# ktiwary2/nerf_pl

Measured on AMD Instinct MI355X. Metric: rays/sec (64c+128f) Blender-lego 400^2 training step, higher is better.
Workload: dtype f16x3

## Files before the change

### __graft_entry__.py

```python
import os
import subprocess
import sys

REPO = os.path.dirname(os.path.abspath(__file__))


def build() -> None:
    jobs = str(min(16, os.cpu_count() or 1))
    subprocess.run(["make", "-C", REPO, "-j", jobs], check=True)
    r = subprocess.run(["make", "-C", REPO, "-j", jobs, "asan"], check=False)
    if r.returncode != 0:
        print(f"build(): optional `make asan` failed (rc {r.returncode}); "
              "tests/test_abi_asan.py will skip", file=sys.stderr)
    if REPO not in sys.path:
        sys.path.insert(0, REPO)
    import nerf_pl_amd
    from nerf_pl_amd import (_lib, _lib_mesh, _lib_mesh_normals, _lib_optim, _lib_posegrad,
                             _lib_raygrad)
    missing = (_lib.missing_symbols() + _lib_mesh.missing_symbols()
               + _lib_mesh_normals.missing_symbols() + _lib_raygrad.missing_symbols()
               + _lib_posegrad.missing_symbols() + _lib_optim.missing_symbols())
    if missing:
        raise RuntimeError(f"libnerf_pl_amd.so lacks {missing}")


def smoke() -> None:
    if REPO not in sys.path:
        sys.path.insert(0, REPO)
    import torch
    from nerf_pl_amd import Embedding, NeRF, ReplayRNG, render_rays
    from nerf_pl_amd.rays import blender_rays
    from oracle import nerf_oracle as O

    dev = torch.device("cuda", 0)
    n_rays, S, I = 64, 32, 32
    rays = blender_rays(16, 1, near=2.0, far=6.0)[:n_rays].contiguous()
    g = torch.Generator().manual_seed(0)
    draws = [torch.rand(n_rays, S, generator=g), torch.randn(n_rays, S, generator=g),
             torch.rand(n_rays, I, generator=g), torch.rand(n_rays, I, generator=g),
             torch.randn(n_rays, S + I, generator=g)]
    params = [O.make_params(1, sigma_bias=0.5), O.make_params(2, sigma_bias=0.5)]
    ocap, cap = {}, {}
    ref = O.render_rays(params, rays, S, False, 1.0, 1.0, I, 32768, False,
                        rng=O.ReplayRNG(draws), capture=ocap)
    models = []
    for p in params:
        m = NeRF()
        m.load_state_dict(p)
        models.append(m.to(dev))
    res = render_rays(models, [Embedding(3, 10), Embedding(3, 4)], rays.to(dev), S, False, 1.0,
                      1.0, I, 32768, False, rng=ReplayRNG(draws), _capture=cap)
    pairs = [(res[k], ref[k]) for k in ref] + \
        [(cap[w], ocap[w]) for w in ("weights_coarse", "weights_fine")]
    worst = max((a.detach().cpu() - b).abs().max().item() for a, b in pairs)
# ... 16 lines not shown
```

### nerf_pl_amd/csrc/mlp_fwd3.hip

```cpp
#include "x3.h"

namespace {

using namespace x3;

constexpr int kHeadBytes = NR_H_SIZE * 4;
constexpr int kHeadDma = (kHeadBytes + 1023) / 1024;
constexpr int kHeadLds = kHeadDma * 1024;
#define NR_PE_REGS (NR_F16 || NR_BF1)
constexpr int kPeQ = 12;
constexpr int kPeBytes = NR_PE_REGS ? 0 : kWaves * kPeQ * 64 * 16;
constexpr int kNS = 2;
constexpr int kBlocks = kWaves;
constexpr int kLdsBytes = kRingBytes + kHeadLds + kPeBytes;
static_assert(kLdsBytes <= 160 * 1024, "LDS budget");

constexpr int kL1 = 0, kL2 = 4, kL3 = 20, kL4 = 36, kL5 = 52, kL6 = 72, kL7 = 88, kL8 = 104;
constexpr int kFinal = 120, kDir = 136, kQAll = 145, kQSigma = 120;

struct FwdTab {
    __host__ __device__ static constexpr int64_t off(int q) {
        return (int64_t)kHeadBytes + (int64_t)q * kSlotBytes;
    }
    __host__ __device__ static constexpr int sg(int q) { return q < kDir ? q / 2 : kDir / 2 + (q - kDir); }
    __host__ __device__ static constexpr int first(int G) { return G < kDir / 2 ? 2 * G : kDir + (G - kDir / 2); }
    __host__ __device__ static constexpr int size(int G) { return G < kDir / 2 ? 2 : 1; }
};
static_assert(FwdTab::off(kQAll) == (NR_F16 ? 2388000 : (NR_BF1 ? 1200160 : 3575840)),
              "packed size must match packing.fwd3_offsets()");

template <bool RELU, int NF, int NS>
__device__ __forceinline__ void head_dot(const f32x4 (&acc)[NF][NS], const float* __restrict__ w,
                                         int g, float (&p)[2]) {
    p[0] = p[1] = 0.f;
#pragma unroll
    for (int F = 0; F < NF; ++F) {
        const f32x4 v = *reinterpret_cast<const f32x4*>(w + 16 * F + 4 * g);
#pragma unroll
        for (int S = 0; S < NS; ++S)
#pragma unroll
            for (int r = 0; r < 4; ++r) p[S] = fmaf(RELU ? relu_keep(acc[F][S][r]) : acc[F][S][r], v[r], p[S]);
    }
#pragma unroll
    for (int S = 0; S < NS; ++S) p[S] = sum_over_groups(p[S]);
}

__device__ __forceinline__ void pe_encode(float (&pe)[16], float px, float py, float pz, int g) {
#pragma unroll
    for (int s = 0; s < 2; ++s)
#pragma unroll
        for (int i = 0; i < 4; ++i) {
            const int m = 4 * (4 * s + g) + i;
            const int k = (m * 11) >> 5;
            const int c = m - 3 * k;
            const float v = c == 0 ? px : (c == 1 ? py : pz);
            float sn, cs;
            sincosf(v * __uint_as_float((uint32_t)(127 + k) << 23), &sn, &cs);
            pe[8 * s + i] = sn;
            pe[8 * s + 4 + i] = cs;
        }
    if (g == 3) {
        pe[10] = px; pe[11] = py; pe[14] = pz; pe[15] = 0.f;
    }
}

__device__ __forceinline__ void pe_gather(float (&pe)[16], const float* __restrict__ row, int g) {
#pragma unroll
    for (int s = 0; s < 2; ++s)
#pragma unroll
        for (int i = 0; i < 4; ++i) {
            const int m = min(4 * (4 * s + g) + i, 29);
            const int k = (m * 11) >> 5;
            const int c = m - 3 * k;
            pe[8 * s + i] = row[3 + 6 * k + c];
            pe[8 * s + 4 + i] = row[6 + 6 * k + c];
        }
    if (g == 3) {
        pe[10] = row[0]; pe[11] = row[1]; pe[14] = row[2]; pe[15] = 0.f;
    }
}

__device__ __forceinline__ void dir_encode(float (&d)[8], float dx, float dy, float dz, int g) {
    const float sc = __uint_as_float((uint32_t)(127 + g) << 23);
    sincosf(dx * sc, &d[0], &d[4]);
    sincosf(dy * sc, &d[1], &d[5]);
    sincosf(dz * sc, &d[2], &d[6]);
    d[3] = g == 0 ? dx : (g == 1 ? dy : (g == 2 ? dz : 0.f));
    d[7] = 0.f;
}

__device__ __forceinline__ void dir_gather(float (&d)[8], const float* __restrict__ row, int g) {
#pragma unroll
    for (int c = 0; c < 3; ++c) {
        d[c] = row[3 + 6 * g + c];
        d[4 + c] = row[6 + 6 * g + c];
    }
    d[3] = g < 3 ? row[min(g, 2)] : 0.f;
    d[7] = 0.f;
}

template <int W, bool ROWS>
__device__ __forceinline__ void store_pe4(const float* v, int s, int jh, int S, int g,
                                          float* __restrict__ blk, int lane) {
    const int T = 2 * s + (g >> 1), gp = 2 * (g & 1) + jh;
#if NR_BF1
    store_slot(f32x4{v[0], v[1], v[2], v[3]}, blk, (T * 2 + S) * 64 + 16 * gp + (lane & 15));
#else
    if constexpr (ROWS)
        *reinterpret_cast<f32x4*>(blk + (16 * S + (lane & 15)) * W + 16 * T + 4 * gp) =
            f32x4{v[0], v[1], v[2], v[3]};
    else
        *reinterpret_cast<f32x4*>(blk + ((T * 2 + S) * 64 + 16 * gp + (lane & 15)) * 4) =
            f32x4{v[0], v[1], v[2], v[3]};
#endif
}

enum FwdMode { FWD_RAYS = 0, FWD_EMB = 1, FWD_PTS = 2 };

template <bool SAVE, bool ROWS>
struct PeSide {
    static constexpr int before(int T) { return SAVE ? (T > 2) + (T > 6) : 0; }
// ... 4 lines not shown
    __device__ __forceinline__ void operator()(GC, int t) const {
        if constexpr (SAVE) {
            if (t == 2 || t == 6) {
                const int u = 2 * GC::value + (t == 6), S = u >> 2, s = (u >> 1) & 1, jh = u & 1;
                store_pe4<64, ROWS>(&pe[S][8 * s + 4 * jh], s, jh, S, g, dst, lane);
            }
        }
    }
};

template <bool SAVE>
struct DirPeSide {
    static constexpr int before(int T) { return SAVE ? T / 2 : 0; }
    const float (&dpe)[kNS][8];
    float* dst;
    int g, lane;
    template <typename GC>
    __device__ __forceinline__ void operator()(GC, int t) const {
        if constexpr (SAVE) {
            if (t & 1) {
                const int u = t >> 1;
                store_pe4<32, true>(&dpe[u >> 1][4 * (u & 1)], 0, u & 1, u >> 1, g, dst, lane);
            }
        }
    }
};

struct Fwd3Args {
    const char* packed;
    const float* pts; const float* rays; const float* z; const float* x;
    int n, spr, xstride;
    float* out; float* save;
    const int32_t* slist; const int32_t* scount;
};

template <bool RELU, bool STORE, bool MASK, bool SIG, bool ROWS = true>
struct AccU {
    static constexpr bool kStores = STORE;
    static constexpr bool kPaired = STORE && ROWS && kRowPair;
    template <typename P> __device__ __forceinline__ void begin(const P&) {}
    const f32x4 (&X)[16][kNS];
    float* dst;
    uint32_t* msk;
    const float* wsig;
    int lane, g;
    float pend[2] = {0.f, 0.f};
    f32x4 held = {0.f, 0.f, 0.f, 0.f};
    uint32_t w[4] = {0u, 0u, 0u, 0u};
    float sig[2] = {0.f, 0.f};
    f32x2 wsg[2][4];
    __device__ __forceinline__ f32x2 wsig_of(int s, int p) const {
        return *reinterpret_cast<const f32x2*>(wsig + 32 * s + 16 * (p >> 1) + 4 * g + 2 * (p & 1));
    }
    __device__ __forceinline__ void preload() {
        if constexpr (SIG)
#pragma unroll
            for (int p = 0; p < 4; ++p) wsg[0][p] = wsig_of(0, p);
    }
    template <typename SC>
    __device__ __forceinline__ void operator()(SC, int sb, int p, float& x0, float& x1) {
        constexpr int s = SC::value;
        x0 = acc_b(X, s, sb, 2 * p);
        x1 = acc_b(X, s, sb, 2 * p + 1);
        if constexpr (RELU) { x0 = relu_unscale(x0); x1 = relu_unscale(x1); }
        else if constexpr (kWScale != 0) { x0 *= kWUnscale; x1 *= kWUnscale; }
        if constexpr (SIG) {
// ... 25 lines not shown
            }
        }
    }
};

template <int N>
struct PeU {
    static constexpr bool kStores = false;
    static constexpr bool kPaired = false;
    template <typename P> __device__ __forceinline__ void begin(const P&) {}
    const float (&pe)[kNS][N];
    template <typename SC>
    __device__ __forceinline__ void operator()(SC, int sb, int p, float& x0, float& x1) const {
        constexpr int s = SC::value;
        x0 = pe[sb][8 * s + 2 * p];
        x1 = pe[sb][8 * s + 2 * p + 1];
    }
};

template <int S = 0, typename GetU>
__device__ __forceinline__ void drain_all(GetU& u) {
    if constexpr (S < 8) {
#pragma unroll
        for (int sb = 0; sb < kNS; ++sb)
#pragma unroll
            for (int p = 0; p < 4; ++p) {
                float x0, x1;
                u(IC<S>(), sb, p, x0, x1);
            }
        drain_all<S + 1>(u);
    }
}

template <int MODE, bool SIGMA_ONLY, bool SAVE, bool LIST = false>
__global__ void __launch_bounds__(64 * kWaves, 1) mlp_fwd3_kernel(Fwd3Args a) {
    constexpr bool EMB = MODE == FWD_EMB;
    constexpr int QEND = SIGMA_ONLY ? kQSigma : kQAll;
    static_assert(!LIST || (SAVE && MODE == FWD_RAYS), "a listed run saves, on the ray path");
    __shared__ __attribute__((aligned(16))) char smem[kLdsBytes];
    const int lane = threadIdx.x & 63;
    const int wave = __builtin_amdgcn_readfirstlane(threadIdx.x >> 6);
    const int g = lane >> 4;
    const int blk = blockIdx.x * kBlocks + wave;
    const int m = LIST ? __builtin_amdgcn_readfirstlane(*a.scount) : a.n;
    if (LIST && (int)blockIdx.x * kBlocks * 32 >= m) return;
    int smp[2];
    bool valid[2];
#pragma unroll
    for (int S = 0; S < kNS; ++S) {
        const int s_raw = blk * 32 + 16 * S + (lane & 15);
        valid[S] = s_raw < m;
        if constexpr (LIST) smp[S] = a.slist[valid[S] ? s_raw : 0];
        else smp[S] = valid[S] ? s_raw : a.n - 1;
    }
    const char* P = a.packed;

    float pe[kNS][16], dg[kNS][8];
    float in[kNS][7];
#pragma unroll
    for (int S = 0; S < kNS; ++S) {
        const int s = smp[S];
        if constexpr (EMB) {
            pe_gather(pe[S], a.x + (size_t)s * a.xstride, g);
            if constexpr (!SIGMA_ONLY) dir_gather(dg[S], a.x + (size_t)s * a.xstride + NR_XYZ_CH, g);
        } else if constexpr (MODE == FWD_PTS) {
#pragma unroll
            for (int c = 0; c < 3; ++c) in[S][c] = a.pts[(size_t)s * 3 + c];
        } else {
            const float* r = a.rays + (size_t)(s / a.spr) * 8;
#pragma unroll
            for (int c = 0; c < 6; ++c) in[S][c] = r[c];
            in[S][6] = a.z[s];
        }
    }

    float* Hs = reinterpret_cast<float*>(smem + kRingBytes);
    const Dma dma = make_dma(P, FwdTab::off(kQAll), smem, wave, lane);
#pragma unroll
    for (int i = wave; i < kHeadDma; i += kWaves)
        __builtin_amdgcn_raw_ptr_buffer_load_lds(
            dma.rsrc, (__attribute__((address_space(3))) void*)(smem + kRingBytes + i * 1024), 16,
            dma.voff, i * 1024, 0, 0);
    prologue<FwdTab, QEND>(dma);
    const float* H = Hs;
    const int nb = (int)nr_blocks_pad(a.n);
    float* const SV = a.save;

    [[maybe_unused]] f32x4* pe_lds =
        reinterpret_cast<f32x4*>(smem + kRingBytes + kHeadLds) + wave * kPeQ * 64 + lane;
#pragma unroll
    for (int S = 0; S < kNS; ++S) {
        if constexpr (MODE == FWD_PTS) {
            pe_encode(pe[S], in[S][0], in[S][1], in[S][2], g);
        } else if constexpr (MODE == FWD_RAYS) {
            const float zz = in[S][6];
            pe_encode(pe[S], nr_add(in[S][0], nr_mul(in[S][3], zz)),
                      nr_add(in[S][1], nr_mul(in[S][4], zz)), nr_add(in[S][2], nr_mul(in[S][5], zz)), g);
            if constexpr (!SIGMA_ONLY) dir_encode(dg[S], in[S][3], in[S][4], in[S][5], g);
        }
    }
#if !NR_PE_REGS
#pragma unroll
    for (int q = 0; q < 8; ++q)
        pe_lds[q * 64] = f32x4{pe[q >> 2][4 * (q & 3)], pe[q >> 2][4 * (q & 3) + 1],
                               pe[q >> 2][4 * (q & 3) + 2], pe[q >> 2][4 * (q & 3) + 3]};
    if constexpr (!SIGMA_ONLY) {
#pragma unroll
        for (int S = 0; S < 2; ++S) {
            pe_lds[(8 + 2 * S) * 64] = f32x4{dg[S][0], dg[S][1], dg[S][2], dg[S][3]};
            pe_lds[(9 + 2 * S) * 64] = f32x4{dg[S][4], dg[S][5], dg[S][6], dg[S][7]};
        }
    }
#endif

    Ahead f0;
    enter<FwdTab, 0, QEND>(smem, lane, f0);

    ActN<kNS> A, B;
    Pieces b[kNS];
    auto hseg = [&](int l) { return SV + nr_sv_h(l, nb) + (size_t)blk * NR_SEGF(256); };
    NoSide none;
    NoNext nonext;
    ZeroInit zero;
    auto bias = [&](int off) { return BiasInit{H + off, g}; };
    constexpr bool kRows = !SIGMA_ONLY;
    using U = AccU<true, SAVE, SAVE, false, kRows>;
    uint32_t* const mblk =
        reinterpret_cast<uint32_t*>(SV + nr_sv_mask(nb)) + (size_t)blk * NR_MASK_LAYERS * 256;
    auto mseg = [&](int l) { return mblk + l * 256; };

    PeU<16> peu{pe};
    split_all(peu, b);
    U u1{A, hseg(0), mseg(0), nullptr, lane, g};
    {
        PeSide<SAVE, kRows> side{pe, SV + (size_t)blk * NR_SEGF(64), g, lane};
        auto bi = bias(NR_H_BIAS(1));
        segment<FwdTab, kL1, 2, 2, QEND, true>(dma, lane, A, peu, u1, bi, side, b, f0);
    }
    U u2{B, hseg(1), mseg(1), nullptr, lane, g};
    { auto bi = bias(NR_H_BIAS(2)); segment<FwdTab, kL2, 8, 2, QEND, true>(dma, lane, B, u1, u2, bi, none, b, f0); }
    U u3{A, hseg(2), mseg(2), nullptr, lane, g};
    { auto bi = bias(NR_H_BIAS(3)); segment<FwdTab, kL3, 8, 2, QEND, true>(dma, lane, A, u2, u3, bi, none, b, f0); }
    float pe5[kNS][16];
#if NR_PE_REGS
#pragma unroll
    for (int S = 0; S < kNS; ++S)
#pragma unroll
        for (int i = 0; i < 16; ++i) pe5[S][i] = pe[S][i];
#else
#pragma unroll
    for (int q = 0; q < 8; ++q) {
        const f32x4 v = pe_lds[q * 64];
#pragma unroll
        for (int e = 0; e < 4; ++e) pe5[q >> 2][4 * (q & 3) + e] = v[e];
    }
#endif
    PeU<16> pe5u{pe5};
    { auto bi = bias(NR_H_BIAS(4)); segment<FwdTab, kL4, 8, 2, QEND, true>(dma, lane, B, u3, pe5u, bi, none, b, f0); }
    U u4{B, hseg(3), mseg(3), nullptr, lane, g};
    { auto bi = bias(NR_H_BIAS(5)); segment<FwdTab, kL5, 2, 2, QEND, true>(dma, lane, A, pe5u, u4, bi, none, b, f0); }
    U u5{A, hseg(4), mseg(4), nullptr, lane, g};
    segment<FwdTab, kL5 + 4, 8, 2, QEND, false>(dma, lane, A, u4, u5, zero, none, b, f0);
    U u6{B, hseg(5), mseg(5), nullptr, lane, g};
    { auto bi = bias(NR_H_BIAS(6)); segment<FwdTab, kL6, 8, 2, QEND, true>(dma, lane, B, u5, u6, bi, none, b, f0); }
    U u7{A, hseg(6), mseg(6), nullptr, lane, g};
    { auto bi = bias(NR_H_BIAS(7)); segment<FwdTab, kL7, 8, 2, QEND, true>(dma, lane, A, u6, u7, bi, none, b, f0); }

    const int Sw = g & 1;
// ... 116 lines not shown

}

#if NR_F16
#define NR_FWD3_BYTES_NAME nr_fwd3_packed_bytes_h3
#elif NR_BF1
#define NR_FWD3_BYTES_NAME nr_fwd3_packed_bytes_b1
#else
#define NR_FWD3_BYTES_NAME nr_fwd3_packed_bytes
#endif
NR_API int64_t NR_FWD3_BYTES_NAME(void) { return FwdTab::off(kQAll); }

NR_API int NR_X3_NAME(nr_pack)(const float* flat, const int32_t* map, int64_t n, const int32_t* head_map,
                      void* out, void* stream) {
    NR_REQUIRE(n == (FwdTab::off(kQAll) - kHeadBytes) / 2, "nr_pack_x3: map has %lld entries, "
               "expected %lld", (long long)n, (long long)((FwdTab::off(kQAll) - kHeadBytes) / 2));
    NR_REQUIRE(flat && map && head_map && out, "nr_pack_x3: null pointer");
    pack3_kernel<<<(unsigned)((n + 255) / 256), 256, 0, (hipStream_t)stream>>>(
        flat, map, n, head_map, reinterpret_cast<char*>(out));
    NR_LAUNCH_CHECK("nr_pack_x3");
    return 0;
}

NR_API int NR_X3_NAME(nr_mlp_fwd)(const void* packed, const float* rays, const float* z, int64_t n,
                         int samples_per_ray, const float* x, int xstride, int sigma_only,
                         float* out, float* save, void* stream) {
    NR_REQUIRE(n >= 0 && n < (int64_t)1 << 31, "nr_mlp_fwd_x3: n=%lld out of range", (long long)n);
    if (n == 0) return 0;
    NR_REQUIRE(packed && out, "nr_mlp_fwd_x3: null packed/out");
    NR_REQUIRE(((uintptr_t)packed & 15) == 0 && ((uintptr_t)out & 15) == 0 &&
                   ((uintptr_t)save & 15) == 0,
               "nr_mlp_fwd_x3: packed/out/save must be 16-byte aligned");
    const bool emb = x != nullptr;
    if (emb) {
        NR_REQUIRE(xstride >= (sigma_only ? NR_XYZ_CH : NR_XYZ_CH + NR_DIR_CH),
                   "nr_mlp_fwd_x3: xstride %d too small", xstride);
    } else {
        NR_REQUIRE(rays && z && samples_per_ray > 0, "nr_mlp_fwd_x3: rays/z/samples_per_ray");
    }
    NR_REQUIRE(!(sigma_only && save && emb),
               "nr_mlp_fwd_x3: a sigma_only run keeps activations only on the ray path");
    Fwd3Args a{reinterpret_cast<const char*>(packed), nullptr, rays, z, x, (int)n,
               samples_per_ray, xstride, out, save};
    const int blocks = (int)((n + 32 * kBlocks - 1) / (32 * kBlocks));
    hipStream_t st = (hipStream_t)stream;
    const bool sv = save != nullptr;
    if (emb) {
        if (sigma_only) mlp_fwd3_kernel<FWD_EMB, true, false><<<blocks, 64 * kWaves, 0, st>>>(a);
        else if (sv) mlp_fwd3_kernel<FWD_EMB, false, true><<<blocks, 64 * kWaves, 0, st>>>(a);
        else mlp_fwd3_kernel<FWD_EMB, false, false><<<blocks, 64 * kWaves, 0, st>>>(a);
    } else {
        if (sigma_only && sv) mlp_fwd3_kernel<FWD_RAYS, true, true><<<blocks, 64 * kWaves, 0, st>>>(a);
        else if (sigma_only) mlp_fwd3_kernel<FWD_RAYS, true, false><<<blocks, 64 * kWaves, 0, st>>>(a);
        else if (sv) mlp_fwd3_kernel<FWD_RAYS, false, true><<<blocks, 64 * kWaves, 0, st>>>(a);
        else mlp_fwd3_kernel<FWD_RAYS, false, false><<<blocks, 64 * kWaves, 0, st>>>(a);
    }
    NR_LAUNCH_CHECK("nr_mlp_fwd_x3");
    return 0;
}

#if !NR_BF1
NR_API int NR_X3_NAME(nr_mlp_fwd_listed)(const void* packed, const float* rays, const float* z,
                                         int64_t n, int samples_per_ray, int sigma_only,
                                         float* save, const int32_t* samples,
                                         const int32_t* count, void* stream) {
    NR_REQUIRE(n >= 0 && n < (int64_t)1 << 31, "nr_mlp_fwd_listed: n=%lld out of range", (long long)n);
    if (n == 0) return 0;
    NR_REQUIRE(packed && rays && z && save && samples && count && samples_per_ray > 0,
               "nr_mlp_fwd_listed: null pointer or samples_per_ray");
    NR_REQUIRE(((uintptr_t)packed & 15) == 0 && ((uintptr_t)save & 15) == 0,
               "nr_mlp_fwd_listed: packed/save must be 16-byte aligned");
    Fwd3Args a{reinterpret_cast<const char*>(packed), nullptr, rays, z, nullptr, (int)n,
               samples_per_ray, 0, nullptr, save, samples, count};
    const int blocks = (int)((n + 32 * kBlocks - 1) / (32 * kBlocks));
    hipStream_t st = (hipStream_t)stream;
    if (sigma_only) mlp_fwd3_kernel<FWD_RAYS, true, true, true><<<blocks, 64 * kWaves, 0, st>>>(a);
    else mlp_fwd3_kernel<FWD_RAYS, false, true, true><<<blocks, 64 * kWaves, 0, st>>>(a);
    NR_LAUNCH_CHECK("nr_mlp_fwd_listed");
    return 0;
// ... 17 lines not shown
```

### nerf_pl_amd/functions.py

```python
from __future__ import annotations

import collections
import functools
import os
import threading
import weakref

import torch

from . import ops, packing
from ._lib import call, stream_of


@functools.lru_cache(maxsize=4)
def _wgrad_workspace(device_index: int, stream: int = 0) -> torch.Tensor:
    from ._lib import lib
    nbytes = int(lib().nr_wgrad_workspace_bytes(0))
    return torch.empty(nbytes // 4, dtype=torch.float32, device=torch.device("cuda", device_index))


SIGMA_TRAIN_KERNELS = os.environ.get("NERF_PL_AMD_SIGMA_TRAIN", "1") != "0"

ACTIVE_SAMPLES = os.environ.get("NERF_PL_AMD_ACTIVE_SAMPLES", "1") != "0"
ACTIVE_ARITHS = ("f16x3", "bf16x6", "fp32")
# ... 22 lines not shown
            return None
        while e.pending and e.pending[0][1].query():
            host, _, n = e.pending.popleft()
            e.frac = int(host[0]) / max(n, 1)
        while len(e.pending) > 16:
            e.pending.popleft()
        return e.frac


def _note_listed(model, sigma_only, count_dev, n):
    host = torch.empty(1, dtype=torch.int32, pin_memory=True)
    host.copy_(count_dev, non_blocking=True)
    ev = torch.cuda.Event()
    ev.record()
    with _LISTED_LOCK:
        per_model = _LISTED.get(model)
        if per_model is None:
            per_model = _LISTED[model] = {}
        per_model.setdefault(sigma_only, _ListedStats()).pending.append((host, ev, n))


ACTIVE_LOG = None

_DEBUG = {} if os.environ.get("NERF_PL_AMD_DEBUG") == "1" else None

_SHAPES = list(packing.param_shapes().items())
_SIGMA_ONLY_UNUSED = {"xyz_encoding_final.weight", "xyz_encoding_final.bias",
                      "dir_encoding.0.weight", "dir_encoding.0.bias",
                      "rgb.0.weight", "rgb.0.bias"}


class _FusedMLP(torch.autograd.Function):
    @staticmethod
    def forward(ctx, model, rays, z, spr, x, sigma_only, *params):
        train = any(ctx.needs_input_grad[6:])
        ray_grad = x is None and (ctx.needs_input_grad[1] or ctx.needs_input_grad[2])
        bwd = train or ray_grad
        if train and sigma_only and x is not None:
            raise NotImplementedError("nerf_pl_amd: training NeRF.forward(x, sigma_only=True) on "
                                      "pre-embedded input is not supported; use render_rays")
        packed_f, packed_b = model.packed(backward=bwd)
        so_train = bwd and sigma_only and SIGMA_TRAIN_KERNELS and x is None
        kern_sigma_only = sigma_only and (not bwd or so_train)
        defer = False
        if bwd and x is None and ACTIVE_SAMPLES and ops.arith_of(packed_b) in ACTIVE_ARITHS:
            if DEFER_SAVE == "all" or (DEFER_SAVE in ("sigma", "auto") and so_train):
                defer = True
            elif DEFER_SAVE == "auto":
                frac = _listed_fraction(model, sigma_only)
                defer = frac is not None and frac < DEFER_AUTO
        model.__dict__["_nr_defer_last"] = defer
        if x is None:
            rays = ops._dev(rays, "rays", 8)
            z = ops._dev(z, "z")
        out, save = ops.mlp_forward(packed_f, rays=rays, z=z, samples_per_ray=spr, x=x,
                                    sigma_only=kern_sigma_only, save=bwd and not defer)
        if _DEBUG is not None and save is not None:
            _DEBUG.setdefault("fwd_saves", []).append((save, out.shape[0], ops.MATH))
        if bwd:
            flat = model.flat_params()
            if defer:
                ctx.save_for_backward(out, rays, z, packed_f, packed_b, flat, *params)
            else:
                ctx.save_for_backward(out, save, packed_f, packed_b, flat, *params,
                                      *((rays, z) if ray_grad else ()))
            ctx.spr = spr
            ctx.train, ctx.ray_grad = train, ray_grad
            ctx.defer = defer
            ctx.sigma_only = sigma_only
            ctx.model = model if DEFER_SAVE == "auto" else None
            ctx.so_kernels = so_train
        if sigma_only and bwd and out.shape[1] == 4:
            out = out[:, 3:4].contiguous()
        return out

    @staticmethod
    def backward(ctx, g_out):
        if ctx.defer:
            out, rays, z, packed_f, packed_b, flat = ctx.saved_tensors[:6]
            n, mode = z.numel(), "_listed"
        else:
            out, save, packed_f, packed_b, flat = ctx.saved_tensors[:5]
            n = out.shape[0]
            mode = "_active" if ACTIVE_SAMPLES and ops.arith_of(packed_b) in ACTIVE_ARITHS else ""
        dev = out.device
        if ctx.sigma_only:
            g4 = torch.zeros(n, 4, device=dev)
            g4[:, 3:4] = g_out
            g_out = g4
# ... 4 lines not shown
        sfx = ("_sigma" if so else "") + mode
        st = stream_of(dev)
        lst = ()
        if mode:
            sl = _sample_list(ctx, g_out, n, st)
            lst = (sl.data_ptr(), sl.data_ptr() + 4 * n)
        if ctx.defer:
            save = torch.empty(ops.save_floats(n), device=dev)
            call(ops.entry("nr_mlp_fwd_listed", packed_f), packed_f.data_ptr(), rays.data_ptr(),
                 z.data_ptr(), n, int(ctx.spr), int(so), save.data_ptr(), *lst, st)
        grad_ws = torch.empty(ops.n_blocks(n) * ops.GRAD_PER_BLOCK, device=dev)
        call(ops.entry("nr_mlp_bwd" + sfx, packed_b), packed_b.data_ptr(), ops.head_ptr(packed_f),
             out.data_ptr(), g_out.data_ptr(), save.data_ptr(), n, grad_ws.data_ptr(), *lst, st)
        gflat = None
        if ctx.train:
            gflat = torch.empty(packing.N_PARAMS, device=dev)
            ws = _wgrad_workspace(dev.index, int(st))
            call(ops.entry("nr_wgrad" + sfx, packed_b), save.data_ptr(), grad_ws.data_ptr(), n,
                 ws.data_ptr(), gflat.data_ptr(), *lst, st)
            if not so:
                _dir_feat(flat, gflat, st)
        g_rays = g_z = None
        if ctx.ray_grad:
            if not ctx.defer:
                rays, z = ctx.saved_tensors[-2:]
            g_rays, g_smp = ops.mlp_ray_gradient(flat, grad_ws, rays, z, int(ctx.spr),
                                                 ops.arith_of(packed_b), so, lst)
            g_rays = g_rays if ctx.needs_input_grad[1] else None
            g_z = g_smp[:, 3] if ctx.needs_input_grad[2] else None
        if _DEBUG is not None:
            _DEBUG.update(save=save, grad_ws=grad_ws, g_out=g_out, gflat=gflat, n=n)
            _DEBUG.setdefault("g_outs", []).append(g_out)
        pgrads = _param_grads(gflat, ctx.sigma_only) if ctx.train else (None,) * len(_SHAPES)
        return (None, g_rays, g_z, None, None, None) + pgrads


def _sample_list(ctx, g_out, n, st):
    sl = torch.empty(n + 1 + 2 * ((n + 31) // 32), dtype=torch.int32, device=g_out.device)
    call("nr_active_samples", g_out.data_ptr(), n, sl.data_ptr(), sl.data_ptr() + 4 * n,
         sl.data_ptr() + 4 * (n + 1), st)
    if ACTIVE_LOG is not None:
        ACTIVE_LOG.append((sl, n))
    if ctx.model is not None:
        _note_listed(ctx.model, ctx.sigma_only, sl[n:n + 1], n)
    return sl


def _dir_feat(flat, gflat, st):
    call("nr_wgrad_dir_feat", flat.data_ptr(), gflat.data_ptr(), st)


def _param_grads(gflat, sigma_only):
    grads, off = [], 0
    for name, shp in _SHAPES:
        k = 1
        for d in shp:
            k *= d
        g = gflat[off:off + k].view(shp)
        off += k
        grads.append(None if (sigma_only and name in _SIGMA_ONLY_UNUSED) else g)
    return tuple(grads)


def mlp_apply(model, *, rays=None, z=None, spr=0, x=None, sigma_only=False):
    if x is not None and x.requires_grad:
        raise NotImplementedError("nerf_pl_amd: gradients w.r.t. the embedded input are not "
                                  "produced (the reference never needs them)")
    params = model.ordered_params()
    if z is not None:
        z = z.reshape(-1)
    ray_grad = x is None and any(t is not None and t.requires_grad for t in (rays, z))
    if not (any(p.requires_grad for p in params) or ray_grad) or not torch.is_grad_enabled():
        packed_f, _ = model.packed()
        out, _ = ops.mlp_forward(packed_f, rays=rays, z=z, samples_per_ray=spr, x=x,
                                 sigma_only=sigma_only)
        return out
    return _FusedMLP.apply(model, rays, z, spr, x, sigma_only, *params)


class _Composite(torch.autograd.Function):

    @staticmethod
    def forward(ctx, raw, z, rays, noise, noise_std, seed, stream, white_back, disp):
        outs = ops.composite_forward(raw, z, rays, noise, noise_std, seed, stream, white_back,
                                     disp=disp)
        ctx.save_for_backward(raw, z, rays, noise if noise is not None else torch.empty(0),
                              *(outs[1:3] if disp else ()))
        ctx.cfg = (noise is not None, noise_std, seed, stream, white_back, disp)
        ctx.mark_non_differentiable(outs[-1])
        ctx.set_materialize_grads(False)
        return outs

    @staticmethod
    def backward(ctx, *g):
        raw, z, rays, noise = ctx.saved_tensors[:4]
        has_noise, noise_std, seed, stream, white_back, disp = ctx.cfg
        noise = noise if has_noise else None
        g_raw = g_z = g_rays = None
        if ctx.needs_input_grad[0]:
            g_raw = ops.composite_backward(raw, z, rays, noise, noise_std, seed, stream,
                                           white_back, *g[:-1], *ctx.saved_tensors[4:], disp=disp)
        if ctx.needs_input_grad[1] or ctx.needs_input_grad[2]:
            g_z, g_rays = ops.composite_ray_gradient(raw, z, rays, noise, noise_std, seed, stream,
                                                     white_back, *g[:-1], *ctx.saved_tensors[4:],
                                                     disp=disp)
            g_z = g_z if ctx.needs_input_grad[1] else None
            g_rays = g_rays if ctx.needs_input_grad[2] else None
        return (g_raw, g_z, g_rays) + (None,) * 6


# ... 56 lines not shown
```

### nerf_pl_amd/ops.py

```python
from __future__ import annotations

import functools
import os

import numpy as np
import torch

from . import packing
from ._lib import call, lib, ptr, stream_of

BLK = 32
MATHS = ("f16x3", "bf16x6", "fp32", "bf16")
MATH = os.environ.get("NERF_PL_AMD_MATH", "f16x3")
if MATH not in MATHS:
    raise ValueError(f"NERF_PL_AMD_MATH must be one of {MATHS}, got {MATH!r}")
SAVE_PER_BLOCK = BLK * (64 + 8 * 256 + 128 + 32) + 9 * 256
SAVE_STATS, STAT_SEGS = 16, 11


_LAYOUT_OK = False
ABI_REVISION = 2


def _check_layout():
    global _LAYOUT_OK
    if not _LAYOUT_OK:
        q = lib().nr_layout_query
        got = (int(q(3)), int(q(4)), int(q(9)))
        want = (SAVE_PER_BLOCK, GRAD_PER_BLOCK, ABI_REVISION)
        if got != want:
            raise RuntimeError(f"nerf_pl_amd: libnerf_pl_amd.so has (save block, grad block, ABI "
                               f"revision) {got}, the package {want}: rebuild the library (make)")
        _LAYOUT_OK = True


def save_floats(n: int) -> int:
    _check_layout()
    nb = n_blocks(n)
    return nb * SAVE_PER_BLOCK + SAVE_STATS + STAT_SEGS * nb
GRAD_PER_BLOCK = BLK * (8 * 256 + 128 + 4)

# ... 98 lines not shown

def pack_fwd_fp32(flat: torch.Tensor, out: torch.Tensor | None = None) -> torch.Tensor:
    m, _ = _maps(flat.device.index)
    out = torch.empty(FWD_PACKED, device=flat.device) if out is None else out
    call("nr_pack", ptr(flat), ptr(m), m.numel(), ptr(out), stream_of(flat.device))
    return out


@functools.lru_cache(maxsize=None)
def _map_bwd3(device_index: int, np_: int = 3):
    return torch.from_numpy(packing.build_bwd3_map(np_)).to(torch.device("cuda", device_index))


def pack_bwd(flat: torch.Tensor, out: torch.Tensor | None = None, math: str | None = None):
    math = math or MATH
    if math in _SUFFIX:
        np_ = packing.NPIECES[math]
        m = _map_bwd3(flat.device.index, np_)
        out = torch.empty(packing.bwd3_bytes(np_), dtype=torch.uint8, device=flat.device) \
            if out is None else out
        call("nr_pack_bwd" + _SUFFIX[math], ptr(flat), ptr(m), m.numel(), ptr(out),
             stream_of(flat.device))
        return out
    return pack_bwd_fp32(flat, out)


def pack_bwd_fp32(flat: torch.Tensor, out: torch.Tensor | None = None) -> torch.Tensor:
    _, m = _maps(flat.device.index)
    out = torch.empty(BWD_PACKED, device=flat.device) if out is None else out
    call("nr_pack", ptr(flat), ptr(m), m.numel(), ptr(out), stream_of(flat.device))
    return out


def mlp_forward(packed: torch.Tensor, *, rays=None, z=None, samples_per_ray=0, x=None,
                sigma_only=False, save=False):
    if x is not None:
        x = _dev(x, "x")
        n, xstride = x.shape[0], x.shape[1]
    else:
        rays = _dev(rays, "rays", 8)
        z = _dev(z, "z")
        n, xstride = z.numel(), 0
    dev = packed.device
    out = torch.empty(n, 1 if sigma_only and not save else 4, device=dev)
    sv = torch.empty(save_floats(n), device=dev) if save else None
    call(entry("nr_mlp_fwd", packed), ptr(packed), ptr(rays), ptr(z), n, int(samples_per_ray),
         ptr(x), xstride, int(sigma_only), ptr(out), ptr(sv), stream_of(dev))
    return out, sv


def sigma_points(packed, pts):
    pts = _dev(pts, "pts", 3)
    out = torch.empty(pts.shape[0], device=pts.device)
    call(entry("nr_mlp_sigma_points", packed), ptr(packed), ptr(pts), pts.shape[0], ptr(out),
         stream_of(pts.device))
    return out


def coarse_z(rays, n_samples, use_disp, perturb, u=None, seed=0):
    rays = _dev(rays, "rays", 8)
    n_rays = rays.shape[0]
    z = torch.empty(n_rays, n_samples, device=rays.device)
    tl = linspace_table(n_samples, rays.device.index)
    call("nr_coarse_z", ptr(rays), ptr(tl), n_rays, n_samples, int(use_disp), float(perturb),
         ptr(u), seed, ptr(z), stream_of(rays.device))
    return z


def composite_forward(raw, z, rays, noise, noise_std, seed, rng_stream, white_back,
                      weights_only=False, disp=False):
    if disp and weights_only:
        raise ValueError("composite_forward: weights_only produces no disparity map")
    z = _dev(z, "z")
    n_rays, S = z.shape
    stride = raw.shape[-1]
    dev = z.device
    opac = torch.empty(n_rays, device=dev)
    w = torch.empty(n_rays, S, device=dev)
# ... 155 lines not shown
```

### nerf_pl_amd/rendering.py

```python
from __future__ import annotations

import functools
import os

import torch

from . import ops
from .functions import coarse_z_apply, composite_apply, merged_z_apply, mlp_apply
from .rng import (STREAM_JITTER, STREAM_NOISE_COARSE, STREAM_NOISE_FINE, STREAM_PERTURB,
                  STREAM_U, PhiloxRNG, TorchRNG)

__all__ = ["render_rays", "sample_pdf"]

FINE_STREAM = os.environ.get("NERF_PL_AMD_FINE_STREAM", "1") != "0"
FINE_STREAM_PRIORITY = int(os.environ.get("NERF_PL_AMD_FINE_STREAM_PRIORITY", "0"))


BEFORE_FINE = []


@functools.lru_cache(maxsize=None)
def _side_stream(device_index: int):
    return torch.cuda.Stream(device=torch.device("cuda", device_index),
                             priority=FINE_STREAM_PRIORITY)
# ... 37 lines not shown
    rng = PhiloxRNG() if rng is None else rng
    n_rays, nb = weights.shape
    w_full = torch.nn.functional.pad(weights.detach(), (1, 1))
    u = rng.rand((n_rays, N_importance), rays.device)
    jit = rng.rand((n_rays, N_importance), rays.device)
    z, _ = ops.sample_pdf(w_full, rays, N_importance, u=u, jitter=jit, seed=rng.seed)
    return z


def render_rays(models, embeddings, rays, N_samples=64, use_disp=False, perturb=0, noise_std=1,
                N_importance=0, chunk=1024 * 32, white_back=False, test_time=False, *, rng=None,
                _capture=None):
    return _render_rays(models, embeddings, rays, N_samples, use_disp, perturb, noise_std,
                        N_importance, chunk, white_back, test_time, rng, _capture)


def _render_rays(models, embeddings, rays, N_samples, use_disp, perturb, noise_std, N_importance,
                 chunk, white_back, test_time, rng, _capture, disp=False, depth_only=False,
                 pipelined=True, empty_ok=False):
    if isinstance(rays, torch.Tensor) and rays.device.type == "cpu":
        if depth_only:
            raise NotImplementedError("nerf_pl_amd.render_rays: depth_only needs a HIP-device batch")
        if rays.dtype != torch.float32:
            raise TypeError(f"rays: expected float32, got {rays.dtype}")
        if rays.dim() != 2 or rays.shape[-1] != 8:
            raise ValueError(f"rays: expected (N, 8), got {tuple(rays.shape)}")
        from .host import render_rays_host
        return render_rays_host(models, embeddings, rays, N_samples, use_disp, perturb, noise_std,
                                N_importance, chunk, white_back, test_time,
                                TorchRNG() if rng is None else rng, _capture, disp=disp)
    del chunk
    fused = _fused_ok(models, embeddings)

    def mlp(model, z, spr, sigma_only=False):
        if fused:
            return mlp_apply(model, rays=rays, z=z, spr=spr, sigma_only=sigma_only)
        return _composable_mlp(model, embeddings, rays, z, spr, sigma_only)

    rays = ops._dev(rays, "rays", 8)
    if not fused and rays.requires_grad and torch.is_grad_enabled():
        raise NotImplementedError(
            "nerf_pl_amd.render_rays: the composable path (a non-default NeRF or Embedding) does "
            "not produce the gradient with respect to the rays; detach them, or use the default "
            "NeRF() with [Embedding(3, 10), Embedding(3, 4)]")
    dev = rays.device
    n_rays = rays.shape[0]
    if n_rays == 0 and not empty_ok:
        raise ValueError("nerf_pl_amd.render_rays: empty ray batch (the reference's "
                         "inference() concatenates an empty chunk list, rendering.py:161)")
    rng = PhiloxRNG() if rng is None else rng
    seed = rng.seed

    def composite(result, level, raw, z, noise, stream):
        rgb, depth, opac, *dmap, w = composite_apply(raw, z, rays, noise, noise_std, seed, stream,
                                                     white_back, disp)
        if rgb is not None:
            result["rgb_" + level] = rgb
        result["depth_" + level] = depth
        result["opacity_" + level] = opac
        if disp:
            result["disp_map_" + level] = dmap[0]
        return w

    u1 = rng.rand((n_rays, N_samples), dev) if perturb > 0 else None
    z_c = coarse_z_apply(rays, N_samples, use_disp, perturb, u=u1, seed=seed)
    noise_c = rng.randn((n_rays, N_samples), dev)

    cap = _capture if _capture is not None else {}
    cap["z_coarse"] = z_c
# ... 5 lines not shown
                                                      STREAM_NOISE_COARSE, white_back,
                                                      weights_only=True)
        result["opacity_coarse"] = opac_c
    else:
        raw_c = mlp(models[0], z_c, N_samples, sigma_only=depth_only)
        w_c = composite(result, "coarse", raw_c, z_c, noise_c, STREAM_NOISE_COARSE)

    cap["weights_coarse"] = w_c
    if N_importance > 0:
        u = rng.rand((n_rays, N_importance), dev)
        jit = rng.rand((n_rays, N_importance), dev)
        z_f = merged_z_apply(z_c, w_c.detach(), rays, N_importance, u, jit, seed)
        cap["z_fine"] = z_f
        s_f = N_samples + N_importance

        fine = {}

        def fine_pass():
            noise_f = rng.randn((n_rays, s_f), dev)
            raw_f = mlp(models[1], z_f, s_f, sigma_only=depth_only)
            w = composite(fine, "fine", raw_f, z_f, noise_f, STREAM_NOISE_FINE)
            return tuple(fine.values()) + (w,)

        while pipelined and BEFORE_FINE:
            BEFORE_FINE.pop(0)()
        if pipelined and FINE_STREAM and torch.is_grad_enabled() and any(
                p.requires_grad for p in models[1].parameters()):
            main = torch.cuda.current_stream(dev)
            side = _side_stream(dev.index)
            side.wait_stream(main)
            with torch.cuda.stream(side):
                outs = fine_pass()
            main.wait_stream(side)
            for t in (rays, z_f):
                t.record_stream(side)
            for t in outs:
                t.record_stream(main)
        else:
            outs = fine_pass()
        cap["weights_fine"] = outs[-1]
        result.update(fine)
    return result


_STREAMS = (STREAM_PERTURB, STREAM_NOISE_COARSE, STREAM_U, STREAM_JITTER, STREAM_NOISE_FINE)
```

Measured before the change: 539,000.

## Precompute positional and direction encodings in separate kernels before the fused MLP

Adds standalone kernels that compute the xyz positional encoding directly into the save buffer's PE segment and a per-ray direction encoding cached across the coarse and fine passes. In f16x3 training mode the fused MLP forward then reads these encoded rows instead of evaluating sincos inline, and it skips storing the PE side output. The intent is to take the transcendental work out of the register- and LDS-heavy MLP kernel and reuse the direction encoding across both passes. The cost is extra kernel launches and extra global memory traffic for writing and re-reading the encoded rows.

```diff
diff --git a/__graft_entry__.py b/__graft_entry__.py
--- a/__graft_entry__.py
+++ b/__graft_entry__.py
@@ -15,11 +15,12 @@
     if REPO not in sys.path:
         sys.path.insert(0, REPO)
     import nerf_pl_amd
-    from nerf_pl_amd import (_lib, _lib_mesh, _lib_mesh_normals, _lib_optim, _lib_posegrad,
-                             _lib_raygrad)
+    from nerf_pl_amd import (_lib, _lib_encode, _lib_mesh, _lib_mesh_normals, _lib_optim,
+                             _lib_posegrad, _lib_raygrad)
     missing = (_lib.missing_symbols() + _lib_mesh.missing_symbols()
                + _lib_mesh_normals.missing_symbols() + _lib_raygrad.missing_symbols()
-               + _lib_posegrad.missing_symbols() + _lib_optim.missing_symbols())
+               + _lib_posegrad.missing_symbols() + _lib_optim.missing_symbols()
+               + _lib_encode.missing_symbols())
     if missing:
         raise RuntimeError(f"libnerf_pl_amd.so lacks {missing}")
 
diff --git a/include/nerf_pl_amd_encode.h b/include/nerf_pl_amd_encode.h
--- /dev/null
+++ b/include/nerf_pl_amd_encode.h
@@ -0,0 +1,21 @@
+#ifndef NERF_PL_AMD_ENCODE_H
+#define NERF_PL_AMD_ENCODE_H
+
+#include <stdint.h>
+
+#ifdef __cplusplus
+extern "C" {
+#endif
+
+#define NR_X_ENCODED (-1)
+
+int nr_encode_dirs(const float* rays, int64_t n_rays, float* out, void* stream);
+
+int nr_encode_points(const float* rays, const float* z, int64_t n, int samples_per_ray,
+                     float* out, void* stream);
+
+#ifdef __cplusplus
+}
+#endif
+
+#endif
diff --git a/nerf_pl_amd/_lib_encode.py b/nerf_pl_amd/_lib_encode.py
--- /dev/null
+++ b/nerf_pl_amd/_lib_encode.py
@@ -0,0 +1,44 @@
+from __future__ import annotations
+
+import ctypes
+
+from . import _lib
+
+_p = ctypes.c_void_p
+_i = ctypes.c_int
+_i64 = ctypes.c_int64
+
+X_ENCODED = -1
+
+SIGNATURES = {
+    "nr_encode_dirs": [_p, _i64, _p, _p],
+    "nr_encode_points": [_p, _p, _i64, _i, _p, _p],
+}
+RESTYPES = {}
+
+_bound = None
+
+
+def lib():
+    global _bound
+    if _bound is None:
+        L = _lib.lib()
+        for name, args in SIGNATURES.items():
+            fn = getattr(L, name, None)
+            if fn is None:
+                continue
+            fn.argtypes = args
+            fn.restype = RESTYPES.get(name, _i)
+        _bound = L
+    return _bound
+
+
+def missing_symbols() -> list:
+    L = lib()
+    return [n for n in SIGNATURES if getattr(L, n, None) is None]
+
+
+def call(name: str, *args) -> None:
+    rc = getattr(lib(), name)(*args)
+    if rc != 0:
+        raise RuntimeError(f"{name} failed (code {rc}): {_lib.last_error()}")
diff --git a/nerf_pl_amd/csrc/encode.h b/nerf_pl_amd/csrc/encode.h
--- /dev/null
+++ b/nerf_pl_amd/csrc/encode.h
@@ -0,0 +1,33 @@
+#pragma once
+#include "common.h"
+
+__device__ __forceinline__ void pe_encode_cell(float* v, float px, float py, float pz, int c) {
+#pragma unroll
+    for (int i = 0; i < 4; ++i) {
+        const int m = 4 * c + i;
+        const int k = (m * 11) >> 5;
+        const int q = m - 3 * k;
+        const float x = q == 0 ? px : (q == 1 ? py : pz);
+        float sn, cs;
+        sincosf(x * __uint_as_float((uint32_t)(127 + k) << 23), &sn, &cs);
+        v[i] = sn;
+        v[4 + i] = cs;
+    }
+    if (c == 7) {
+        v[2] = px; v[3] = py; v[6] = pz; v[7] = 0.f;
+    }
+}
+
+__device__ __forceinline__ void pe_encode(float (&pe)[16], float px, float py, float pz, int g) {
+#pragma unroll
+    for (int s = 0; s < 2; ++s) pe_encode_cell(&pe[8 * s], px, py, pz, 4 * s + g);
+}
+
+__device__ __forceinline__ void dir_encode(float (&d)[8], float dx, float dy, float dz, int g) {
+    const float sc = __uint_as_float((uint32_t)(127 + g) << 23);
+    sincosf(dx * sc, &d[0], &d[4]);
+    sincosf(dy * sc, &d[1], &d[5]);
+    sincosf(dz * sc, &d[2], &d[6]);
+    d[3] = g == 0 ? dx : (g == 1 ? dy : (g == 2 ? dz : 0.f));
+    d[7] = 0.f;
+}
diff --git a/nerf_pl_amd/csrc/encode.hip b/nerf_pl_amd/csrc/encode.hip
--- /dev/null
+++ b/nerf_pl_amd/csrc/encode.hip
@@ -0,0 +1,68 @@
+#include "encode.h"
+#include "layout.h"
+
+namespace {
+
+__global__ void __launch_bounds__(256) encode_dirs_kernel(const float* __restrict__ rays,
+                                                          int64_t n_rays,
+                                                          float* __restrict__ out) {
+    const int64_t t = (int64_t)blockIdx.x * 256 + threadIdx.x;
+    if (t >= n_rays * 4) return;
+    const int64_t r = t >> 2;
+    const int g = (int)(t & 3);
+    const float* ray = rays + r * 8;
+    float d[8];
+    dir_encode(d, ray[3], ray[4], ray[5], g);
+    f32x4* o = reinterpret_cast<f32x4*>(out + r * 32 + 8 * g);
+    o[0] = f32x4{d[0], d[1], d[2], d[3]};
+    o[1] = f32x4{d[4], d[5], d[6], d[7]};
+}
+
+__global__ void __launch_bounds__(256) encode_points_kernel(const float* __restrict__ rays,
+                                                            const float* __restrict__ z,
+                                                            int64_t n, int spr, int64_t rows,
+                                                            float* __restrict__ out) {
+    const int64_t t = (int64_t)blockIdx.x * 256 + threadIdx.x;
+    if (t >= rows * 8) return;
+    const int64_t row = t >> 3;
+    const int c = (int)(t & 7);
+    const int64_t s = row < n ? row : n - 1;
+    const float* ray = rays + (s / spr) * 8;
+    const float zz = z[s];
+    float v[8];
+    pe_encode_cell(v, nr_add(ray[0], nr_mul(ray[3], zz)),
+                   nr_add(ray[1], nr_mul(ray[4], zz)), nr_add(ray[2], nr_mul(ray[5], zz)), c);
+    f32x4* o = reinterpret_cast<f32x4*>(out + row * 64 + 8 * c);
+    o[0] = f32x4{v[0], v[1], v[2], v[3]};
+    o[1] = f32x4{v[4], v[5], v[6], v[7]};
+}
+
+}
+
+NR_API int nr_encode_dirs(const float* rays, int64_t n_rays, float* out, void* stream) {
+    NR_REQUIRE(n_rays >= 0 && n_rays < (int64_t)1 << 31, "nr_encode_dirs: n_rays=%lld out of range",
+               (long long)n_rays);
+    if (n_rays == 0) return 0;
+    NR_REQUIRE(rays && out, "nr_encode_dirs: null pointer");
+    NR_REQUIRE(((uintptr_t)out & 15) == 0, "nr_encode_dirs: out must be 16-byte aligned");
+    const int64_t blocks = (n_rays * 4 + 255) / 256;
+    encode_dirs_kernel<<<(unsigned)blocks, 256, 0, (hipStream_t)stream>>>(rays, n_rays, out);
+    NR_LAUNCH_CHECK("nr_encode_dirs");
+    return 0;
+}
+
+NR_API int nr_encode_points(const float* rays, const float* z, int64_t n, int samples_per_ray,
+                            float* out, void* stream) {
+    NR_REQUIRE(n >= 0 && n < (int64_t)1 << 31, "nr_encode_points: n=%lld out of range",
+               (long long)n);
+    if (n == 0) return 0;
+    NR_REQUIRE(rays && z && out, "nr_encode_points: null pointer");
+    NR_REQUIRE(samples_per_ray > 0, "nr_encode_points: samples_per_ray=%d", samples_per_ray);
+    NR_REQUIRE(((uintptr_t)out & 15) == 0, "nr_encode_points: out must be 16-byte aligned");
+    const int64_t rows = nr_blocks_pad(n) * NR_BLK;
+    const int64_t blocks = (rows * 8 + 255) / 256;
+    encode_points_kernel<<<(unsigned)blocks, 256, 0, (hipStream_t)stream>>>(rays, z, n,
+                                                                            samples_per_ray, rows, out);
+    NR_LAUNCH_CHECK("nr_encode_points");
+    return 0;
+}
diff --git a/nerf_pl_amd/csrc/mlp_fwd3.hip b/nerf_pl_amd/csrc/mlp_fwd3.hip
--- a/nerf_pl_amd/csrc/mlp_fwd3.hip
+++ b/nerf_pl_amd/csrc/mlp_fwd3.hip
@@ -1,3 +1,4 @@
+#include "encode.h"
 #include "x3.h"
 
 namespace {
@@ -45,25 +46,6 @@
     for (int S = 0; S < NS; ++S) p[S] = sum_over_groups(p[S]);
 }
 
-__device__ __forceinline__ void pe_encode(float (&pe)[16], float px, float py, float pz, int g) {
-#pragma unroll
-    for (int s = 0; s < 2; ++s)
-#pragma unroll
-        for (int i = 0; i < 4; ++i) {
-            const int m = 4 * (4 * s + g) + i;
-            const int k = (m * 11) >> 5;
-            const int c = m - 3 * k;
-            const float v = c == 0 ? px : (c == 1 ? py : pz);
-            float sn, cs;
-            sincosf(v * __uint_as_float((uint32_t)(127 + k) << 23), &sn, &cs);
-            pe[8 * s + i] = sn;
-            pe[8 * s + 4 + i] = cs;
-        }
-    if (g == 3) {
-        pe[10] = px; pe[11] = py; pe[14] = pz; pe[15] = 0.f;
-    }
-}
-
 __device__ __forceinline__ void pe_gather(float (&pe)[16], const float* __restrict__ row, int g) {
 #pragma unroll
     for (int s = 0; s < 2; ++s)
@@ -78,15 +60,6 @@
     if (g == 3) {
         pe[10] = row[0]; pe[11] = row[1]; pe[14] = row[2]; pe[15] = 0.f;
     }
-}
-
-__device__ __forceinline__ void dir_encode(float (&d)[8], float dx, float dy, float dz, int g) {
-    const float sc = __uint_as_float((uint32_t)(127 + g) << 23);
-    sincosf(dx * sc, &d[0], &d[4]);
-    sincosf(dy * sc, &d[1], &d[5]);
-    sincosf(dz * sc, &d[2], &d[6]);
-    d[3] = g == 0 ? dx : (g == 1 ? dy : (g == 2 ? dz : 0.f));
-    d[7] = 0.f;
 }
 
 __device__ __forceinline__ void dir_gather(float (&d)[8], const float* __restrict__ row, int g) {
@@ -157,6 +130,7 @@
     int n, spr, xstride;
     float* out; float* save;
     const int32_t* slist; const int32_t* scount;
+    const float* enc_dir;
 };
 
 template <bool RELU, bool STORE, bool MASK, bool SIG, bool ROWS = true>
@@ -248,11 +222,13 @@
     }
 }
 
-template <int MODE, bool SIGMA_ONLY, bool SAVE, bool LIST = false>
+template <int MODE, bool SIGMA_ONLY, bool SAVE, bool LIST = false, bool ENC = false>
 __global__ void __launch_bounds__(64 * kWaves, 1) mlp_fwd3_kernel(Fwd3Args a) {
     constexpr bool EMB = MODE == FWD_EMB;
     constexpr int QEND = SIGMA_ONLY ? kQSigma : kQAll;
     static_assert(!LIST || (SAVE && MODE == FWD_RAYS), "a listed run saves, on the ray path");
+    static_assert(!ENC || (MODE == FWD_RAYS && !LIST && SAVE && !SIGMA_ONLY && !NR_BF1),
+                  "encoded rows: the full graph's sample-major fp32 save layout, by sample");
     __shared__ __attribute__((aligned(16))) char smem[kLdsBytes];
     const int lane = threadIdx.x & 63;
     const int wave = __builtin_amdgcn_readfirstlane(threadIdx.x >> 6);
@@ -282,6 +258,25 @@
         } else if constexpr (MODE == FWD_PTS) {
 #pragma unroll
             for (int c = 0; c < 3; ++c) in[S][c] = a.pts[(size_t)s * 3 + c];
+        } else if constexpr (ENC) {
+            const f32x4* row = reinterpret_cast<const f32x4*>(
+                a.save + ((size_t)blk * 32 + 16 * S + (lane & 15)) * 64 + 8 * g);
+#pragma unroll
+            for (int u = 0; u < 2; ++u)
+#pragma unroll
+                for (int h = 0; h < 2; ++h) {
+                    const f32x4 v = row[8 * u + h];
+#pragma unroll
+                    for (int e = 0; e < 4; ++e) pe[S][8 * u + 4 * h + e] = v[e];
+                }
+            const f32x4* dr = reinterpret_cast<const f32x4*>(
+                a.enc_dir + (size_t)(s / a.spr) * 32 + 8 * g);
+#pragma unroll
+            for (int h = 0; h < 2; ++h) {
+                const f32x4 v = dr[h];
+#pragma unroll
+                for (int e = 0; e < 4; ++e) dg[S][4 * h + e] = v[e];
+            }
         } else {
             const float* r = a.rays + (size_t)(s / a.spr) * 8;
 #pragma unroll
@@ -308,7 +303,7 @@
     for (int S = 0; S < kNS; ++S) {
         if constexpr (MODE == FWD_PTS) {
             pe_encode(pe[S], in[S][0], in[S][1], in[S][2], g);
-        } else if constexpr (MODE == FWD_RAYS) {
+        } else if constexpr (MODE == FWD_RAYS && !ENC) {
             const float zz = in[S][6];
             pe_encode(pe[S], nr_add(in[S][0], nr_mul(in[S][3], zz)),
                       nr_add(in[S][1], nr_mul(in[S][4], zz)), nr_add(in[S][2], nr_mul(in[S][5], zz)), g);
@@ -349,7 +344,7 @@
     split_all(peu, b);
     U u1{A, hseg(0), mseg(0), nullptr, lane, g};
     {
-        PeSide<SAVE, kRows> side{pe, SV + (size_t)blk * NR_SEGF(64), g, lane};
+        PeSide<SAVE && !ENC, kRows> side{pe, SV + (size_t)blk * NR_SEGF(64), g, lane};
         auto bi = bias(NR_H_BIAS(1));
         segment<FwdTab, kL1, 2, 2, QEND, true>(dma, lane, A, peu, u1, bi, side, b, f0);
     }
@@ -532,9 +527,19 @@
                    ((uintptr_t)save & 15) == 0,
                "nr_mlp_fwd_x3: packed/out/save must be 16-byte aligned");
     const bool emb = x != nullptr;
+    const bool enc = !emb && xstride == -1;
     if (emb) {
         NR_REQUIRE(xstride >= (sigma_only ? NR_XYZ_CH : NR_XYZ_CH + NR_DIR_CH),
                    "nr_mlp_fwd_x3: xstride %d too small", xstride);
+    } else if (enc) {
+        NR_REQUIRE(NR_F16, "nr_mlp_fwd_x3: encoded rows (NR_X_ENCODED) are read by nr_mlp_fwd_h3 only");
+        NR_REQUIRE(z && rays && samples_per_ray > 0, "nr_mlp_fwd_x3: encoded rows/samples_per_ray");
+        NR_REQUIRE(((uintptr_t)rays & 15) == 0,
+                   "nr_mlp_fwd_x3: encoded rows must be 16-byte aligned");
+        NR_REQUIRE(!sigma_only && save,
+                   "nr_mlp_fwd_x3: encoded rows are read by the full graph's saving forward only");
+        NR_REQUIRE(z == save,
+                   "nr_mlp_fwd_x3: the xyz rows are read from the save buffer's PE segment");
     } else {
         NR_REQUIRE(rays && z && samples_per_ray > 0, "nr_mlp_fwd_x3: rays/z/samples_per_ray");
     }
@@ -545,6 +550,13 @@
     const int blocks = (int)((n + 32 * kBlocks - 1) / (32 * kBlocks));
     hipStream_t st = (hipStream_t)stream;
     const bool sv = save != nullptr;
+#if NR_F16
+    if (enc) {
+        a.rays = a.z = nullptr;
+        a.enc_dir = rays;
+        mlp_fwd3_kernel<FWD_RAYS, false, true, false, true><<<blocks, 64 * kWaves, 0, st>>>(a);
+    } else
+#endif
     if (emb) {
         if (sigma_only) mlp_fwd3_kernel<FWD_EMB, true, false><<<blocks, 64 * kWaves, 0, st>>>(a);
         else if (sv) mlp_fwd3_kernel<FWD_EMB, false, true><<<blocks, 64 * kWaves, 0, st>>>(a);
diff --git a/nerf_pl_amd/functions.py b/nerf_pl_amd/functions.py
--- a/nerf_pl_amd/functions.py
+++ b/nerf_pl_amd/functions.py
@@ -78,8 +78,8 @@
 
 class _FusedMLP(torch.autograd.Function):
     @staticmethod
-    def forward(ctx, model, rays, z, spr, x, sigma_only, *params):
-        train = any(ctx.needs_input_grad[6:])
+    def forward(ctx, model, rays, z, spr, x, sigma_only, dir_cache, *params):
+        train = any(ctx.needs_input_grad[7:])
         ray_grad = x is None and (ctx.needs_input_grad[1] or ctx.needs_input_grad[2])
         bwd = train or ray_grad
         if train and sigma_only and x is not None:
@@ -100,7 +100,8 @@
             rays = ops._dev(rays, "rays", 8)
             z = ops._dev(z, "z")
         out, save = ops.mlp_forward(packed_f, rays=rays, z=z, samples_per_ray=spr, x=x,
-                                    sigma_only=kern_sigma_only, save=bwd and not defer)
+                                    sigma_only=kern_sigma_only, save=bwd and not defer,
+                                    dir_cache=dir_cache)
         if _DEBUG is not None and save is not None:
             _DEBUG.setdefault("fwd_saves", []).append((save, out.shape[0], ops.MATH))
         if bwd:
@@ -171,7 +172,7 @@
             _DEBUG.update(save=save, grad_ws=grad_ws, g_out=g_out, gflat=gflat, n=n)
             _DEBUG.setdefault("g_outs", []).append(g_out)
         pgrads = _param_grads(gflat, ctx.sigma_only) if ctx.train else (None,) * len(_SHAPES)
-        return (None, g_rays, g_z, None, None, None) + pgrads
+        return (None, g_rays, g_z, None, None, None, None) + pgrads
 
 
 def _sample_list(ctx, g_out, n, st):
@@ -201,7 +202,7 @@
     return tuple(grads)
 
 
-def mlp_apply(model, *, rays=None, z=None, spr=0, x=None, sigma_only=False):
+def mlp_apply(model, *, rays=None, z=None, spr=0, x=None, sigma_only=False, dir_cache=None):
     if x is not None and x.requires_grad:
         raise NotImplementedError("nerf_pl_amd: gradients w.r.t. the embedded input are not "
                                   "produced (the reference never needs them)")
@@ -212,9 +213,9 @@
     if not (any(p.requires_grad for p in params) or ray_grad) or not torch.is_grad_enabled():
         packed_f, _ = model.packed()
         out, _ = ops.mlp_forward(packed_f, rays=rays, z=z, samples_per_ray=spr, x=x,
-                                 sigma_only=sigma_only)
+                                 sigma_only=sigma_only, dir_cache=dir_cache)
         return out
-    return _FusedMLP.apply(model, rays, z, spr, x, sigma_only, *params)
+    return _FusedMLP.apply(model, rays, z, spr, x, sigma_only, dir_cache, *params)
 
 
 class _Composite(torch.autograd.Function):
diff --git a/nerf_pl_amd/ops.py b/nerf_pl_amd/ops.py
--- a/nerf_pl_amd/ops.py
+++ b/nerf_pl_amd/ops.py
@@ -6,7 +6,7 @@
 import numpy as np
 import torch
 
-from . import packing
+from . import _lib_encode, packing
 from ._lib import call, lib, ptr, stream_of
 
 BLK = 32
@@ -171,8 +171,35 @@
     return out
 
 
+ENCODE_KERNEL = os.environ.get("NERF_PL_AMD_ENCODE_KERNEL", "1") != "0"
+
+
+def encode_enabled(math: str | None = None) -> bool:
+    return ENCODE_KERNEL and (math or MATH) == "f16x3"
+
+
+def encode_dirs(rays: torch.Tensor) -> torch.Tensor:
+    rays = _dev(rays, "rays", 8)
+    _lib_encode.lib()
+    out = torch.empty(rays.shape[0], 32, device=rays.device)
+    call("nr_encode_dirs", ptr(rays), rays.shape[0], ptr(out), stream_of(rays.device))
+    return out
+
+
+def encode_points(rays, z, samples_per_ray, out=None) -> torch.Tensor:
+    rays = _dev(rays, "rays", 8)
+    z = _dev(z, "z")
+    n = z.numel()
+    _lib_encode.lib()
+    if out is None:
+        out = torch.empty(n_blocks(n) * BLK, 64, device=rays.device)
+    call("nr_encode_points", ptr(rays), ptr(z), n, int(samples_per_ray), ptr(out),
+         stream_of(rays.device))
+    return out
+
+
 def mlp_forward(packed: torch.Tensor, *, rays=None, z=None, samples_per_ray=0, x=None,
-                sigma_only=False, save=False):
+                sigma_only=False, save=False, dir_cache=None):
     if x is not None:
         x = _dev(x, "x")
         n, xstride = x.shape[0], x.shape[1]
@@ -183,6 +210,13 @@
     dev = packed.device
     out = torch.empty(n, 1 if sigma_only and not save else 4, device=dev)
     sv = torch.empty(save_floats(n), device=dev) if save else None
+    if x is None and save and not sigma_only and encode_enabled(arith_of(packed)):
+        encode_points(rays, z, samples_per_ray, out=sv)
+        if dir_cache is None:
+            dir_cache = []
+        if not dir_cache:
+            dir_cache.append(encode_dirs(rays))
+        rays, z, xstride = dir_cache[0], sv, _lib_encode.X_ENCODED
     call(entry("nr_mlp_fwd", packed), ptr(packed), ptr(rays), ptr(z), n, int(samples_per_ray),
          ptr(x), xstride, int(sigma_only), ptr(out), ptr(sv), stream_of(dev))
     return out, sv
diff --git a/nerf_pl_amd/rendering.py b/nerf_pl_amd/rendering.py
--- a/nerf_pl_amd/rendering.py
+++ b/nerf_pl_amd/rendering.py
@@ -93,9 +93,12 @@
     del chunk
     fused = _fused_ok(models, embeddings)
 
+    enc_dirs = []
+
     def mlp(model, z, spr, sigma_only=False):
         if fused:
-            return mlp_apply(model, rays=rays, z=z, spr=spr, sigma_only=sigma_only)
+            return mlp_apply(model, rays=rays, z=z, spr=spr, sigma_only=sigma_only,
+                             dir_cache=enc_dirs)
         return _composable_mlp(model, embeddings, rays, z, spr, sigma_only)
 
     rays = ops._dev(rays, "rays", 8)
@@ -167,7 +170,7 @@
             with torch.cuda.stream(side):
                 outs = fine_pass()
             main.wait_stream(side)
-            for t in (rays, z_f):
+            for t in (rays, z_f, *enc_dirs):
                 t.record_stream(side)
             for t in outs:
                 t.record_stream(main)
```

Result: no change. 542,000 (median of 6 runs) (+0.6%).
